# W298/Surtr

Measured on AMD Instinct MI355X. Metric: fragments/sec, higher is better.
Workload: dtype f32

## Files before the change

surtr_amd/csrc/surtr_hip.hip:

```cpp
#include <algorithm>
#include <cmath>
#include <cstdio>
#include <cstdlib>
#include <cstring>
#include <string>
#include <type_traits>
#include <vector>

#include "surtr_ctx.h"
#include "small_clip.h"
#ifndef SC_RESUME
#define SC_RESUME 1
#endif
#include "literal_clip.h"
#include "wave_clip.h"
#include "prep_sorted.h"

template <uint32_t LV, uint32_t LH>
struct alignas(16) LdsTopoT
{
    static_assert(LV % 16 == 0 && LH % 8 == 0, "clip_image copies 16-byte words into these arrays");
    static constexpr uint32_t kLV = LV, kLH = LH;
    alignas(16) uint16_t loff[LV];
    alignas(16) uint8_t llen[LV];
// ... 1812 lines not shown
    refit_fragments(HullFirst4{}, frags, counts, pool, A, forder, cap_frags, frag_status, piece_cpos, piece_cvo);
}

__global__ __launch_bounds__(SURTR_LANES) void k_refit_n(FragRec* __restrict__ frags, const surtr_counts* __restrict__ counts,
                                                      ScratchPool pool, Arena A, const uint32_t* __restrict__ forder, uint32_t cap_frags,
                                                      uint32_t* __restrict__ frag_status, const float* __restrict__ piece_cpos,
                                                      const uint32_t* __restrict__ piece_cvo, uint32_t limit, uint32_t* __restrict__ hull_ws)
{
    refit_fragments(HullLimited{limit, A.capV, hull_ws}, frags, counts, pool, A, forder, cap_frags, frag_status, piece_cpos, piece_cvo);
}

__global__ __launch_bounds__(SURTR_LANES) void k_hull_probe(const float* __restrict__ pts, uint32_t n, uint32_t limit, uint32_t* __restrict__ ws,
                                                         float* __restrict__ normals, uint32_t* __restrict__ out )
{
    __shared__ RhLds H;
    __shared__ ArgF slotF[SURTR_NWAVE];
    __shared__ ArgD slotD[SURTR_NWAVE];
    const int rc = rh_build(pts, n, n < limit ? n : limit, (float*)ws, ws + n, H, slotF, slotD);
    if (rc == 0)
        for (uint32_t i = threadIdx.x; i < 3u * H.nLive; i += group_size()) normals[i] = (&H.nrm[0][0])[i];
    if (threadIdx.x == 0) { out[0] = (uint32_t)rc; out[1] = rc == 0 ? H.nLive : 0u; }
}


__device__ __forceinline__ bool on_right(const float* a, const float* b, const float* c, float nx, float ny, float nz)
{
    const float ux = b[0] - a[0], uy = b[1] - a[1], uz = b[2] - a[2];
    const float wx = c[0] - a[0], wy = c[1] - a[1], wz = c[2] - a[2];
    const float cx = uy * wz - uz * wy, cy = uz * wx - ux * wz, cz = ux * wy - uy * wx;
    return dot3(cx, cy, cz, nx, ny, nz) > 0.f;
}

template <class LP>
__device__ __attribute__((always_inline)) static inline uint32_t ear_clip_face(const float* pos, const LP* loop, int N, int32_t* tmp, uint32_t* out)
{
    if (N <= 2) return 0;
    if (N == 3) { out[0] = loop[0]; out[1] = loop[1]; out[2] = loop[2]; return 3; }
    const float* A0 = pos + 3 * loop[0]; const float* B0 = pos + 3 * loop[1]; const float* C0 = pos + 3 * loop[2];
    float nx, ny, nz;
    {
        const float ux = B0[0] - A0[0], uy = B0[1] - A0[1], uz = B0[2] - A0[2];
        const float wx = C0[0] - A0[0], wy = C0[1] - A0[1], wz = C0[2] - A0[2];
        nx = uy * wz - uz * wy; ny = uz * wx - ux * wz; nz = ux * wy - uy * wx;
    }
    {
        float sx = 0.f, sy = 0.f, sz = 0.f;
        for (int v = 0; v < N; ++v)
        {
            const float* p = pos + 3 * loop[v]; const float* q = pos + 3 * loop[(v + 1) % N];
            const float ux = p[0] - A0[0], uy = p[1] - A0[1], uz = p[2] - A0[2];
            const float wx = q[0] - A0[0], wy = q[1] - A0[1], wz = q[2] - A0[2];
            sx = sx + (uy * wz - uz * wy); sy = sy + (uz * wx - ux * wz); sz = sz + (ux * wy - uy * wx);
        }
        if (dot3(sx, sy, sz, nx, ny, nz) < 0.f) { nx = -nx; ny = -ny; nz = -nz; }
    }
    int32_t* prv = tmp; int32_t* nxt = tmp + N; int32_t* rfx = tmp + 2 * N;
    for (int i = 0; i < N; ++i) { prv[i] = (i + N - 1) % N; nxt[i] = (i + 1) % N; }
    for (int i = 0; i < N; ++i)
        rfx[i] = on_right(pos + 3 * loop[prv[i]], pos + 3 * loop[i], pos + 3 * loop[nxt[i]], nx, ny, nz) ? 0 : 1;
    int skipped = 0, left = N, cur = 0;
    uint32_t at = 0;
    while (left > 3)
    {
        const int p = prv[cur], n = nxt[cur];
        bool ear = rfx[cur] == 0;
        if (ear)
        {
            const float* a = pos + 3 * loop[p]; const float* b = pos + 3 * loop[cur]; const float* c = pos + 3 * loop[n];
            for (int r = 0; r < N && ear; ++r)
            {
                if (!rfx[r]) continue;
                if (r == p || r == n) continue;
                const float* q = pos + 3 * loop[r];
                if ((q[0] == a[0] && q[1] == a[1] && q[2] == a[2]) || (q[0] == b[0] && q[1] == b[1] && q[2] == b[2])) continue;
                if (!on_right(a, b, q, nx, ny, nz)) continue;
                if (!on_right(b, c, q, nx, ny, nz)) continue;
                if (!on_right(c, a, q, nx, ny, nz)) continue;
                ear = false;
            }
        }
        if (ear)
        {
            out[at] = loop[p]; out[at + 1] = loop[cur]; out[at + 2] = loop[n];
            nxt[p] = n; prv[n] = p;
            const int adj[2] = {p, n};
            for (int k = 0; k < 2; ++k)
            {
                const int v = adj[k];
                if (!rfx[v]) continue;
                rfx[v] = on_right(pos + 3 * loop[prv[v]], pos + 3 * loop[v], pos + 3 * loop[nxt[v]], nx, ny, nz) ? 0 : 1;
            }
            at += 3; --left; skipped = 0;
        }
        else if (++skipped > left) return 0;
        cur = n;
    }
    out[at] = loop[prv[cur]]; out[at + 1] = loop[cur]; out[at + 2] = loop[nxt[cur]];
    return at + 3;
}

template <class LP>
__device__ __attribute__((always_inline)) static inline uint32_t ear_clip_small(const float* pos, const LP* loop, int N, uint32_t* out)
{
    if (N <= 2) return 0;
    if (N == 3) { out[0] = loop[0]; out[1] = loop[1]; out[2] = loop[2]; return 3; }
    auto P = [&](int i) -> const float* { return pos + 3 * (int)loop[i]; };
    const float* A0 = P(0); const float* B0 = P(1); const float* C0 = P(2);
    float nx, ny, nz;
    {
        const float ux = B0[0] - A0[0], uy = B0[1] - A0[1], uz = B0[2] - A0[2];
        const float wx = C0[0] - A0[0], wy = C0[1] - A0[1], wz = C0[2] - A0[2];
        nx = uy * wz - uz * wy; ny = uz * wx - ux * wz; nz = ux * wy - uy * wx;
    }
    {
        float sx = 0.f, sy = 0.f, sz = 0.f;
        for (int v = 0; v < N; ++v)
        {
            const float* p = P(v); const float* q = P((v + 1) % N);
            const float ux = p[0] - A0[0], uy = p[1] - A0[1], uz = p[2] - A0[2];
            const float wx = q[0] - A0[0], wy = q[1] - A0[1], wz = q[2] - A0[2];
            sx = sx + (uy * wz - uz * wy); sy = sy + (uz * wx - ux * wz); sz = sz + (ux * wy - uy * wx);
        }
        if (dot3(sx, sy, sz, nx, ny, nz) < 0.f) { nx = -nx; ny = -ny; nz = -nz; }
    }
    uint32_t prv = 0, nxt = 0, rfx = 0;
    auto get = [](uint32_t w, int i) -> int { return (int)((w >> (4 * i)) & 15u); };
    auto put = [](uint32_t& w, int i, int v) { w = (w & ~(15u << (4 * i))) | ((uint32_t)v << (4 * i)); };
    for (int i = 0; i < N; ++i) { put(prv, i, (i + N - 1) % N); put(nxt, i, (i + 1) % N); }
    for (int i = 0; i < N; ++i)
        if (!on_right(P(get(prv, i)), P(i), P(get(nxt, i)), nx, ny, nz)) rfx |= 1u << i;
    int skipped = 0, left = N, cur = 0;
    uint32_t at = 0;
    while (left > 3)
    {
        const int p = get(prv, cur), n = get(nxt, cur);
        bool ear = ((rfx >> cur) & 1u) == 0u;
        if (ear)
        {
            const float* a = P(p); const float* b = P(cur); const float* c = P(n);
            for (int r = 0; r < N && ear; ++r)
            {
                if (!((rfx >> r) & 1u)) continue;
                if (r == p || r == n) continue;
                const float* q = P(r);
                if ((q[0] == a[0] && q[1] == a[1] && q[2] == a[2]) || (q[0] == b[0] && q[1] == b[1] && q[2] == b[2])) continue;
                if (!on_right(a, b, q, nx, ny, nz)) continue;
                if (!on_right(b, c, q, nx, ny, nz)) continue;
                if (!on_right(c, a, q, nx, ny, nz)) continue;
                ear = false;
            }
        }
        if (ear)
        {
            out[at] = loop[p]; out[at + 1] = loop[cur]; out[at + 2] = loop[n];
            put(nxt, p, n); put(prv, n, p);
            const int adj[2] = {p, n};
            for (int k = 0; k < 2; ++k)
            {
                const int v = adj[k];
                if (!((rfx >> v) & 1u)) continue;
                if (on_right(P(get(prv, v)), P(v), P(get(nxt, v)), nx, ny, nz)) rfx &= ~(1u << v);
            }
            at += 3; --left; skipped = 0;
        }
        else if (++skipped > left) return 0;
        cur = n;
    }
    out[at] = loop[get(prv, cur)]; out[at + 1] = loop[cur]; out[at + 2] = loop[get(nxt, cur)];
    return at + 3;
}

#ifndef SURTR_EAR_WAVE_MAX
#define SURTR_EAR_WAVE_MAX 256u
#endif
#if SURTR_LANES == 64
template <class LP>
__device__ __attribute__((always_inline)) static inline uint32_t ear_clip_face_wave(const float* pos, const LP* loop, int N, uint32_t* out)
{
    const int lane = (int)lane_id();
    const bool mine = lane < N;
    const int32_t vid = (int32_t)loop[mine ? lane : 0];
    const float x = pos[3 * vid], y = pos[3 * vid + 1], z = pos[3 * vid + 2];
#ifdef SURTR_EAR_SHFL
#define EAR_BCAST(v, i) __shfl(v, i, 64)
#else
#define EAR_BCAST(v, i) lane_bcast(v, (uint32_t)(i))
#endif
    auto bx = [&](int i) { return EAR_BCAST(x, i); };
    auto by = [&](int i) { return EAR_BCAST(y, i); };
    auto bz = [&](int i) { return EAR_BCAST(z, i); };
    const float ax0 = bx(0), ay0 = by(0), az0 = bz(0);
    float nx, ny, nz;
    {
        const float ux = bx(1) - ax0, uy = by(1) - ay0, uz = bz(1) - az0;
        const float wx = bx(2) - ax0, wy = by(2) - ay0, wz = bz(2) - az0;
        nx = uy * wz - uz * wy; ny = uz * wx - ux * wz; nz = ux * wy - uy * wx;
    }
    {
        float sx = 0.f, sy = 0.f, sz = 0.f;
        for (int v = 0; v < N; ++v)
        {
            const int q = (v + 1) % N;
            const float ux = bx(v) - ax0, uy = by(v) - ay0, uz = bz(v) - az0;
            const float wx = bx(q) - ax0, wy = by(q) - ay0, wz = bz(q) - az0;
            sx = sx + (uy * wz - uz * wy); sy = sy + (uz * wx - ux * wz); sz = sz + (ux * wy - uy * wx);
        }
        if (dot3(sx, sy, sz, nx, ny, nz) < 0.f) { nx = -nx; ny = -ny; nz = -nz; }
    }
    int prv = (lane + N - 1) % N, nxt = (lane + 1) % N;
    auto right_of = [&](float ax, float ay, float az, float bx_, float by_, float bz_, float cx, float cy, float cz) {
        const float ux = bx_ - ax, uy = by_ - ay, uz = bz_ - az;
        const float wx = cx - ax, wy = cy - ay, wz = cz - az;
        const float kx = uy * wz - uz * wy, ky = uz * wx - ux * wz, kz = ux * wy - uy * wx;
        return dot3(kx, ky, kz, nx, ny, nz) > 0.f;
    };
    bool rfx = false;
    {
        const float px_ = __shfl(x, prv, 64), py_ = __shfl(y, prv, 64), pz_ = __shfl(z, prv, 64);
        const float qx = __shfl(x, nxt, 64), qy = __shfl(y, nxt, 64), qz = __shfl(z, nxt, 64);
        rfx = mine && !right_of(px_, py_, pz_, x, y, z, qx, qy, qz);
    }
    int skipped = 0, left = N, cur = 0;
    uint32_t at = 0;
    while (left > 3)
    {
        const int p = EAR_BCAST(prv, cur), n = EAR_BCAST(nxt, cur);
        const bool cur_reflex = EAR_BCAST((int)rfx, cur) != 0;
        bool ear = !cur_reflex;
        if (ear)
        {
            const float ax = bx(p), ay = by(p), az = bz(p);
            const float cx_ = bx(cur), cy_ = by(cur), cz_ = bz(cur);
            const float ex = bx(n), ey = by(n), ez = bz(n);
            bool inside = false;
            if (mine && rfx && lane != p && lane != n)
            {
                const bool same = (x == ax && y == ay && z == az) || (x == cx_ && y == cy_ && z == cz_);
                if (!same)
                    inside = right_of(ax, ay, az, cx_, cy_, cz_, x, y, z) && right_of(cx_, cy_, cz_, ex, ey, ez, x, y, z) &&
                             right_of(ex, ey, ez, ax, ay, az, x, y, z);
            }
            ear = __ballot(inside) == 0ull;
        }
        if (ear)
        {
            if (lane == 0) { out[at] = (uint32_t)loop[p]; out[at + 1] = (uint32_t)loop[cur]; out[at + 2] = (uint32_t)loop[n]; }
            if (lane == p) nxt = n;
            if (lane == n) prv = p;
            const int np = EAR_BCAST(prv, p), nn = EAR_BCAST(nxt, n);
            const float npx = bx(np), npy = by(np), npz = bz(np), nnx = bx(nn), nny = by(nn), nnz = bz(nn);
            const float ppx = bx(p), ppy = by(p), ppz = bz(p), qqx = bx(n), qqy = by(n), qqz = bz(n);
            if (lane == p && rfx) rfx = !right_of(npx, npy, npz, x, y, z, qqx, qqy, qqz);
            if (lane == n && rfx) rfx = !right_of(ppx, ppy, ppz, x, y, z, nnx, nny, nnz);
            at += 3; --left; skipped = 0;
        }
        else if (++skipped > left) return 0;
        cur = n;
    }
    {
        const int p = EAR_BCAST(prv, cur), n = EAR_BCAST(nxt, cur);
        if (lane == 0) { out[at] = (uint32_t)loop[p]; out[at + 1] = (uint32_t)loop[cur]; out[at + 2] = (uint32_t)loop[n]; }
    }
    return at + 3;
}

template <int K, class LP>
__device__ __attribute__((noinline)) static uint32_t ear_clip_face_wave_k(const float* pos, const LP* loop, int N, uint32_t* out)
{
    const int lane = (int)lane_id();
    float x[K], y[K], z[K]; int prv[K], nxt[K]; bool rfx[K], mine[K];
#pragma unroll
    for (int j = 0; j < K; ++j)
    {
        const int v = lane + 64 * j;
        mine[j] = v < N;
        const int32_t vid = (int32_t)loop[mine[j] ? v : 0];
        x[j] = pos[3 * vid]; y[j] = pos[3 * vid + 1]; z[j] = pos[3 * vid + 2];
        prv[j] = (v + N - 1) % N; nxt[j] = (v + 1) % N; rfx[j] = false;
    }
    auto bf = [&](const float (&a)[K], int i) -> float {
        const int jj = i >> 6; const uint32_t l = (uint32_t)(i & 63);
        float r = lane_bcast(a[0], l);
#pragma unroll
        for (int j = 1; j < K; ++j) { const float t = lane_bcast(a[j], l); r = jj == j ? t : r; }
        return r;
    };
    auto bi = [&](const int (&a)[K], int i) -> int {
        const int jj = i >> 6; const uint32_t l = (uint32_t)(i & 63);
        int r = lane_bcast(a[0], l);
#pragma unroll
        for (int j = 1; j < K; ++j) { const int t = lane_bcast(a[j], l); r = jj == j ? t : r; }
        return r;
    };
    auto bb = [&](const bool (&a)[K], int i) -> bool {
        const int jj = i >> 6; const uint32_t l = (uint32_t)(i & 63);
        int r = lane_bcast((int)a[0], l);
#pragma unroll
        for (int j = 1; j < K; ++j) { const int t = lane_bcast((int)a[j], l); r = jj == j ? t : r; }
        return r != 0;
    };
    const float ax0 = bf(x, 0), ay0 = bf(y, 0), az0 = bf(z, 0);
    float nx, ny, nz;
    {
        const float ux = bf(x, 1) - ax0, uy = bf(y, 1) - ay0, uz = bf(z, 1) - az0;
        const float wx = bf(x, 2) - ax0, wy = bf(y, 2) - ay0, wz = bf(z, 2) - az0;
        nx = uy * wz - uz * wy; ny = uz * wx - ux * wz; nz = ux * wy - uy * wx;
    }
    {
        float sx = 0.f, sy = 0.f, sz = 0.f;
        float px_ = ax0, py_ = ay0, pz_ = az0;
        for (int v = 0; v < N; ++v)
        {
            const int q = (v + 1) % N;
            const float qx = bf(x, q), qy = bf(y, q), qz = bf(z, q);
            const float ux = px_ - ax0, uy = py_ - ay0, uz = pz_ - az0;
            const float wx = qx - ax0, wy = qy - ay0, wz = qz - az0;
            sx = sx + (uy * wz - uz * wy); sy = sy + (uz * wx - ux * wz); sz = sz + (ux * wy - uy * wx);
            px_ = qx; py_ = qy; pz_ = qz;
        }
        if (dot3(sx, sy, sz, nx, ny, nz) < 0.f) { nx = -nx; ny = -ny; nz = -nz; }
    }
    auto right_of = [&](float ax, float ay, float az, float bx_, float by_, float bz_, float cx, float cy, float cz) {
        const float ux = bx_ - ax, uy = by_ - ay, uz = bz_ - az;
        const float wx = cx - ax, wy = cy - ay, wz = cz - az;
        const float kx = uy * wz - uz * wy, ky = uz * wx - ux * wz, kz = ux * wy - uy * wx;
        return dot3(kx, ky, kz, nx, ny, nz) > 0.f;
    };
#pragma unroll
    for (int j = 0; j < K; ++j)
    {
        float pxv = 0.f, pyv = 0.f, pzv = 0.f, qxv = 0.f, qyv = 0.f, qzv = 0.f;
#pragma unroll
        for (int s2 = 0; s2 < K; ++s2)
        {
            const float tx = __shfl(x[s2], prv[j] & 63, 64), ty = __shfl(y[s2], prv[j] & 63, 64), tz = __shfl(z[s2], prv[j] & 63, 64);
            if ((prv[j] >> 6) == s2) { pxv = tx; pyv = ty; pzv = tz; }
            const float ux = __shfl(x[s2], nxt[j] & 63, 64), uy = __shfl(y[s2], nxt[j] & 63, 64), uz = __shfl(z[s2], nxt[j] & 63, 64);
            if ((nxt[j] >> 6) == s2) { qxv = ux; qyv = uy; qzv = uz; }
        }
        rfx[j] = mine[j] && !right_of(pxv, pyv, pzv, x[j], y[j], z[j], qxv, qyv, qzv);
    }
    auto set_i = [&](int (&a)[K], int i, int val) {
#pragma unroll
        for (int j = 0; j < K; ++j) if (lane == (i & 63) && (i >> 6) == j) a[j] = val;
    };
    int skipped = 0, left = N, cur = 0;
    uint32_t at = 0;
    while (left > 3)
    {
        const int p = bi(prv, cur), n = bi(nxt, cur);
        bool ear = !bb(rfx, cur);
        if (ear)
        {
            const float ax = bf(x, p), ay = bf(y, p), az = bf(z, p);
            const float cx_ = bf(x, cur), cy_ = bf(y, cur), cz_ = bf(z, cur);
            const float ex = bf(x, n), ey = bf(y, n), ez = bf(z, n);
            bool inside = false;
#pragma unroll
            for (int j = 0; j < K; ++j)
            {
                const int v = lane + 64 * j;
                if (mine[j] && rfx[j] && v != p && v != n)
                {
                    const bool same = (x[j] == ax && y[j] == ay && z[j] == az) || (x[j] == cx_ && y[j] == cy_ && z[j] == cz_);
                    if (!same && right_of(ax, ay, az, cx_, cy_, cz_, x[j], y[j], z[j]) && right_of(cx_, cy_, cz_, ex, ey, ez, x[j], y[j], z[j]) &&
                        right_of(ex, ey, ez, ax, ay, az, x[j], y[j], z[j])) inside = true;
                }
            }
            ear = __ballot(inside) == 0ull;
        }
        if (ear)
        {
            if (lane == 0) { out[at] = (uint32_t)loop[p]; out[at + 1] = (uint32_t)loop[cur]; out[at + 2] = (uint32_t)loop[n]; }
            set_i(nxt, p, n);
            set_i(prv, n, p);
            const int np = bi(prv, p), nn = bi(nxt, n);
            const float npx = bf(x, np), npy = bf(y, np), npz = bf(z, np), nnx = bf(x, nn), nny = bf(y, nn), nnz = bf(z, nn);
            const float ppx = bf(x, p), ppy = bf(y, p), ppz = bf(z, p), qqx = bf(x, n), qqy = bf(y, n), qqz = bf(z, n);
#pragma unroll
            for (int j = 0; j < K; ++j)
            {
                const int v = lane + 64 * j;
                if (v == p && rfx[j]) rfx[j] = !right_of(npx, npy, npz, x[j], y[j], z[j], qqx, qqy, qqz);
                if (v == n && rfx[j]) rfx[j] = !right_of(ppx, ppy, ppz, x[j], y[j], z[j], nnx, nny, nnz);
            }
            at += 3; --left; skipped = 0;
        }
        else if (++skipped > left) return 0;
        cur = n;
    }
    {
        const int p = bi(prv, cur), n = bi(nxt, cur);
        if (lane == 0) { out[at] = (uint32_t)loop[p]; out[at + 1] = (uint32_t)loop[cur]; out[at + 2] = (uint32_t)loop[n]; }
    }
    return at + 3;
}
#endif

__global__ __launch_bounds__(SURTR_WG) __attribute__((amdgpu_waves_per_eu(4, 8))) void k_faces(FragRec* __restrict__ frags, const surtr_counts* __restrict__ counts,
                                                    FaceScratch FS, uint2* __restrict__ blkpool, uint32_t blk_per_wg,
                                                    Arena A, const uint32_t* __restrict__ forder, uint32_t cap_frags,
                                                    uint32_t fan, uint32_t* __restrict__ face_n, uint32_t* __restrict__ face_off,
                                                    int32_t* __restrict__ face_idx, uint32_t* __restrict__ frag_status,
                                                    const uint32_t* __restrict__ take_list, uint32_t* __restrict__ push_list)
{
    __shared__ Shared sh;
#ifndef SURTR_FL_V
#define SURTR_FL_V 1024
#define SURTR_FL_H 4096
#endif
    constexpr uint32_t FL_V = SURTR_FL_V, FL_H = SURTR_FL_H, FL_J = SURTR_FL_H / 2u;
    __shared__ uint16_t f_loff[FL_V]; __shared__ uint16_t f_llen[FL_V]; __shared__ uint16_t f_nbr[FL_H];
    struct IrrLds { uint8_t vis[FL_H]; uint32_t cov[FL_H]; };
    struct JumpLds { uint16_t k0[FL_J], k1[FL_J], x0[FL_J], x1[FL_J], d1[FL_J]; };
    struct EarLds { float pos[3 * FL_V]; uint16_t loop[FL_J]; };
    union FacesLds { IrrLds irr; JumpLds jmp; EarLds ear; };
    static_assert(sizeof(EarLds) <= sizeof(IrrLds), "the ear staging reuses the bytes of the face search");
    static_assert(sizeof(JumpLds) <= sizeof(IrrLds), "the pointer-jumping arrays fit the bytes of the irregular path");
    __shared__ FacesLds FU;
    uint8_t* const f_vis = FU.irr.vis; uint32_t* const f_cov = FU.irr.cov;
// ... 21 lines not shown
        const uint32_t f = sh.misc[7];
        if (f >= nf) break;
        FragRec fr = frags[f];
        const uint32_t n = fr.mv_n, H = fr.mh_n;
        STAMP_DECL;
#ifdef SURTR_STAMP
        const unsigned long long frag_t0 = __builtin_readcyclecounter();
        if (tid == 0) for (int q = 0; q < 16; ++q) sh.ph[q] = 0;
#endif
        if (H > HF)
        {
            if (tid == 0)
            {
                if (push_list != nullptr) push_list[atomicAdd(&A.cursors[CUR_FACES2_N], 1u)] = f;
                else atomicMax(&A.cursors[CUR_STATUS], (uint32_t)SURTR_E_CAPACITY);
            }
            continue;
        }
        const float* pos = A.pos + 3 * (size_t)fr.mv_off;
        const uint32_t* loff = A.loff + fr.mv_off; const uint32_t* llen = A.llen + fr.mv_off;
        const int32_t* nbr = A.nbr + fr.mh_off;
        const bool topo_lds = n <= FL_V && H <= FL_H && n < 0xFFFFu;
        const bool jump_lds = topo_lds && H <= FL_J;
        if (tid == 0) sh.flagBad = 0;
        if (topo_lds)
        {
            for (uint32_t v = tid; v < n; v += group_size()) { f_loff[v] = (uint16_t)(loff[v] - fr.mh_off); f_llen[v] = (uint16_t)llen[v]; }
            for (uint32_t e = tid; e < H; e += group_size()) f_nbr[e] = (uint16_t)nbr[e];
        }
        __syncthreads();
        auto gLO = [&](uint32_t v) -> uint32_t { return loff[v] - fr.mh_off; };
        auto gLN = [&](uint32_t v) -> uint32_t { return llen[v]; };
        auto lLO = [&](uint32_t v) -> uint32_t { return f_loff[v]; };
        auto lLN = [&](uint32_t v) -> uint32_t { return f_llen[v]; };
        auto successors = [&](auto LO, auto LN, const auto* NB, auto* NX, auto* KEY, int32_t* copy) {
            typedef typename std::remove_reference<decltype(NX[0])>::type XT;
            bool dup = false;
            for (uint32_t v = tid; v < n; v += group_size())
            {
                const uint32_t lo = LO(v), len = LN(v);
                for (uint32_t s = 0; s < len; ++s)
                {
                    const uint32_t b = (uint32_t)NB[lo + s];
                    for (uint32_t s2 = 0; s2 < s; ++s2) if ((uint32_t)NB[lo + s2] == b) dup = true;
                    const uint32_t lb = LO(b), nbq = LN(b);
                    uint32_t q = 0;
                    while (q < nbq && (uint32_t)NB[lb + q] != v) ++q;
// ... 157 lines not shown
                if (lensum > HF) return false;
                if (!irregular && lensum != H) pinched = true;
                const uint32_t nb = pinched ? 0u : (H + SURTR_LANES - 1u) >> SURTR_LSH;
                for (uint32_t b = wave_id(); b < nb; b += group_waves())
                {
                    const uint32_t e = (b << SURTR_LSH) + lane_id();
                    uint2 c = make_uint2(0u, 0u);
                    if (e < H) c = ownfn(e);
                    const uint2 ex = wave_excl2(c);
                    if (e < H && c.x)
                    {
                        const uint32_t fi = blk[b].x + ex.x, lo = blk[b].y + ex.y;
                        int32_t* loop = loopbuf + lo;
                        const uint32_t start = vertex_of(e);
                        uint32_t prev = start, curv = (uint32_t)NB[e];
                        uint32_t len = 1; loop[0] = (int32_t)start;
                        while (curv != start && len < c.y)
                        {
                            loop[len++] = (int32_t)curv;
                            const uint32_t nx = (uint32_t)face_next(NB + LO(curv), LN(curv), prev);
                            prev = curv; curv = nx;
                        }
                        faceLo[fi] = (int32_t)lo; faceLen[fi] = (int32_t)len;
                    }
                }
                return true;
            };
            auto owners_ranked = [&]() -> bool {
                auto vertex_of = [&](uint32_t e) -> uint32_t {
                    uint32_t lo_v = 0, hi_v = n;
                    while (hi_v - lo_v > 1) { const uint32_t mid = (lo_v + hi_v) >> 1; if (f_loff[mid] <= e) lo_v = mid; else hi_v = mid; }
                    return lo_v;
                };
                bool bad = false;
                for (uint32_t e = tid; e < H; e += group_size())
                {
                    const uint32_t t = (uint32_t)nxA[e], o = own16[e];
                    if (t >= H || own16[t] != o) { bad = true; continue; }
                    const uint32_t want = o == e ? 0u : (t == o ? 1u : (uint32_t)dist16[t] + 1u);
                    if ((uint32_t)dist16[e] != want) bad = true;
                }
                for (uint32_t v = tid; v < n; v += group_size())
                {
                    const uint32_t lo = f_loff[v], len = f_llen[v];
                    for (uint32_t s1 = 1; s1 < len; ++s1)
                        for (uint32_t s2 = 0; s2 < s1; ++s2) if (own16[lo + s1] == own16[lo + s2]) bad = true;
                }
                if (bad) sh.flagBad = 3;
                __syncthreads();
                if (sh.flagBad == 3) { pinched = true; return true; }
                auto ownfn = [&](uint32_t e) -> uint2 {
                    if ((uint32_t)own16[e] != e) return make_uint2(0u, 0u);
                    return make_uint2(1u, (uint32_t)dist16[(uint32_t)nxA[e]] + 1u);
                };
                scan_blocks(H, blk, sh, ownfn, nfaces, lensum);
                if (lensum != H) { pinched = true; return true; }
                uint16_t* lo_of = free16a; uint16_t* len_of = free16b;
                const uint32_t nb = (H + SURTR_LANES - 1u) >> SURTR_LSH;
                for (uint32_t b = wave_id(); b < nb; b += group_waves())
                {
                    const uint32_t e = (b << SURTR_LSH) + lane_id();
                    uint2 c = make_uint2(0u, 0u);
                    if (e < H) c = ownfn(e);
                    const uint2 ex = wave_excl2(c);
                    if (e < H && c.x)
                    {
                        const uint32_t fi = blk[b].x + ex.x, lo = blk[b].y + ex.y;
                        faceLo[fi] = (int32_t)lo; faceLen[fi] = (int32_t)c.y;
                        lo_of[e] = (uint16_t)lo; len_of[e] = (uint16_t)c.y;
                    }
                }
                __syncthreads();
                for (uint32_t e = tid; e < H; e += group_size())
                {
                    const uint32_t o = own16[e], d = dist16[e];
                    loopbuf[(uint32_t)lo_of[o] + (d == 0u ? 0u : (uint32_t)len_of[o] - d)] = (int32_t)vertex_of(e);
                }
                return true;
            };
            bool ok;
            if (own16 != nullptr && dist16 != nullptr) ok = owners_ranked();
            else if (own16 != nullptr) ok = owners(lLO, lLN, f_nbr, [&](uint32_t e) { return (uint32_t)own16[e] == e; });
            else if (topo_lds) ok = owners(lLO, lLN, f_nbr, [&](uint32_t e) { return kc[e] == (int32_t)e; });
            else ok = owners(gLO, gLN, nbr, [&](uint32_t e) { return kc[e] == (int32_t)e; });
            if (!ok) { failed = true; break; }
        }
        else
        {
            if (staged) { for (uint32_t e = tid; e < H; e += group_size()) f_vis[e] = 0; }
            else for (uint32_t e = tid; e < H; e += group_size()) keyA[e] = 0;
            __syncthreads();
// ... 6 lines not shown
                };
                uint32_t nfc = 0, lo = 0; bool bad = false;
                for (uint32_t i = 0; i < n && !bad; ++i)
                {
                    const uint32_t li = LO(i), ni = LN(i);
                    for (uint32_t s = 0; s < ni && !bad; ++s)
                    {
                        const uint32_t adj = NB[li + s];
                        if (visited[slot_of(i, adj)]) continue;
                        if (lo + 1 > HF || nfc >= HF) { bad = true; break; }
                        uint32_t len = 1; loopbuf[lo] = (int32_t)i;
                        uint32_t prev = i, curv = adj;
                        while (curv != i)
                        {
                            visited[slot_of(prev, curv)] = 1;
                            if (lo + len >= HF || len > H) { bad = true; break; }
                            loopbuf[lo + len++] = (int32_t)curv;
                            const uint32_t nx = face_next(NB + LO(curv), LN(curv), prev);
                            prev = curv; curv = nx;
                        }
                        if (bad) break;
                        visited[slot_of(prev, curv)] = 1;
                        faceLo[nfc] = (int32_t)lo; faceLen[nfc] = (int32_t)len; ++nfc; lo += len;
                    }
                }
                sh.misc[0] = nfc; sh.misc[1] = lo; sh.misc[2] = bad ? 1u : 0u;
            };
            if (tid == 0)
            {
                if (staged) extract([&](uint32_t v) { return (uint32_t)f_loff[v]; }, [&](uint32_t v) { return (uint32_t)f_llen[v]; }, f_nbr, f_vis);
                else extract([&](uint32_t v) { return loff[v] - fr.mh_off; }, [&](uint32_t v) { return llen[v]; }, nbr, keyA);
            }
            __syncthreads();
            nfaces = sh.misc[0]; lensum = sh.misc[1];
            const bool bad = sh.misc[2] != 0;
            __syncthreads();
            if (bad) { failed = true; break; }
        }
        __syncthreads();
        if (!pinched) break;
        irregular = true;
        if (tid == 0) sh.flagBad = 0;
        __syncthreads();
        }
        if (failed)
        {
            if (tid == 0)
            {
                frags[f].idx_off = 0; frags[f].idx_n = 0;
                if (frag_status == nullptr || atomicExch(&frag_status[f], (uint32_t)SURTR_E_TOPOLOGY) == 0u) atomicAdd(&A.cursors[CUR_FLAGGED_FRAGS], 1u);
            }
            continue;
        }
        if (face_n != nullptr)
        {
            for (uint32_t fi = tid; fi < nfaces; fi += group_size()) face_off[fi] = (uint32_t)faceLo[fi];
            for (uint32_t e = tid; e < lensum; e += group_size()) face_idx[e] = loopbuf[e];
            if (tid == 0) { face_off[nfaces] = lensum; face_n[0] = nfaces; face_n[1] = lensum; }
        }
        STAMP(62);
        const bool ear_lds = !fan && n <= FL_V && lensum <= FL_J;
        __syncthreads();
        if (ear_lds)
        {
            for (uint32_t i = tid; i < 3u * n; i += group_size()) FU.ear.pos[i] = pos[i];
            for (uint32_t e = tid; e < lensum; e += group_size()) FU.ear.loop[e] = (uint16_t)loopbuf[e];
            __syncthreads();
        }
        if (fan)
        {
            for (uint32_t fi = tid; fi < nfaces; fi += group_size())
            {
                const uint32_t lo = (uint32_t)faceLo[fi], len = (uint32_t)faceLen[fi];
                uint32_t* out = tri + 3u * (size_t)lo;
                const int32_t* loop = loopbuf + lo;
                uint32_t at = 0;
                for (uint32_t v = 1; v + 1u < len; ++v) { out[at] = (uint32_t)loop[0]; out[at + 1] = (uint32_t)loop[v]; out[at + 2] = (uint32_t)loop[v + 1]; at += 3u; }
                fcnt[fi] = at;
            }
        }
#if SURTR_LANES == 64
        for (uint32_t f0 = 0; f0 < (fan ? 0u : nfaces); f0 += SURTR_LANES)
        {
            const uint32_t fl = f0 + lane_id();
            uint32_t mylo = 0, mylen = 0;
            if (fl < nfaces) { mylo = (uint32_t)faceLo[fl]; mylen = (uint32_t)faceLen[fl]; }
            unsigned long long todo = __ballot(mylen >= 5u && mylen <= SURTR_EAR_WAVE_MAX);
            for (uint32_t ord = 0; todo != 0ull; todo &= todo - 1ull, ++ord)
            {
                if (ord % group_waves() != wave_id()) continue;
                const uint32_t src = (uint32_t)__builtin_ctzll(todo);
                const uint32_t lo = lane_bcast(mylo, src), len = lane_bcast(mylen, src);
                uint32_t cnt;
                if (len > 64u) cnt = ear_clip_face_wave_k<SURTR_EAR_WAVE_MAX / 64>(pos, (const int32_t*)loopbuf + lo, (int)len, tri + 3u * (size_t)lo);
                else if (ear_lds) cnt = ear_clip_face_wave((const float*)FU.ear.pos, (const uint16_t*)FU.ear.loop + lo, (int)len, tri + 3u * (size_t)lo);
                else cnt = ear_clip_face_wave(pos, (const int32_t*)loopbuf + lo, (int)len, tri + 3u * (size_t)lo);
                if (lane_id() == 0) fcnt[f0 + src] = cnt;
            }
        }
        __syncthreads();
        STAMP(63);
#endif
        for (uint32_t fi = tid; fi < (fan ? 0u : nfaces); fi += group_size())
        {
            const uint32_t lo = (uint32_t)faceLo[fi], len = (uint32_t)faceLen[fi];
#if SURTR_LANES == 64
            if (len >= 5u && len <= SURTR_EAR_WAVE_MAX) continue;
#endif
            uint32_t* out = tri + 3u * (size_t)lo;
            uint32_t cnt = 0u;
            if (len >= 3u && len <= 8u)
                cnt = ear_lds ? ear_clip_small((const float*)FU.ear.pos, (const uint16_t*)FU.ear.loop + lo, (int)len, out)
                              : ear_clip_small(pos, (const int32_t*)loopbuf + lo, (int)len, out);
            else if (len > 8u) cnt = ear_clip_face(pos, (const int32_t*)loopbuf + lo, (int)len, eartmp + 3 * (size_t)lo, out);
            fcnt[fi] = cnt;
#ifdef SURTR_STAMP
            if (len > 64u) { atomicAdd(&g_stamp[66], 1ull); atomicAdd(&g_stamp[67], (unsigned long long)len); }
#endif
        }
        __syncthreads();
        STAMP(64);
        auto cntfn = [&](uint32_t fi) -> uint2 { return make_uint2(fcnt[fi], 0u); };
        uint32_t nidx = 0, dum = 0;
        scan_blocks(nfaces, blk, sh, cntfn, nidx, dum);
        if (tid == 0) sh.misc[0] = atomicAdd(&A.cursors[CUR_I], nidx);
        __syncthreads();
        const uint32_t ioff = sh.misc[0];
        if ((uint64_t)ioff + nidx > A.capI) { if (tid == 0) atomicMax(&A.cursors[CUR_STATUS], (uint32_t)SURTR_E_CAPACITY); continue; }
        {
            const uint32_t nb = (nfaces + SURTR_LANES - 1u) >> SURTR_LSH;
            for (uint32_t b = wave_id(); b < nb; b += group_waves())
            {
                const uint32_t fi = (b << SURTR_LSH) + lane_id();
                uint2 c = make_uint2(0u, 0u);
                if (fi < nfaces) c = cntfn(fi);
                const uint2 ex = wave_excl2(c);
                if (fi < nfaces && c.x)
                {
                    const uint32_t* src = tri + 3u * (size_t)(uint32_t)faceLo[fi];
                    uint32_t* dst = A.idx + ioff + blk[b].x + ex.x;
                    for (uint32_t q = 0; q < c.x; ++q) dst[q] = src[q];
                }
            }
        }
        if (tid == 0) { frags[f].idx_off = ioff; frags[f].idx_n = nidx; }
        STAMP(65);
#ifdef SURTR_STAMP
        if (tid == 0)
        {
            const unsigned long long d = __builtin_readcyclecounter() - frag_t0;
            int bkt = 0; while ((d >> bkt) > 1 && bkt < 40) ++bkt; bkt = bkt < 12 ? 0 : bkt - 12; if (bkt > 15) bkt = 15;
            atomicAdd(&g_stamp2[32 + bkt], 1ull); atomicAdd(&g_stamp2[51], d);
            for (int q = 0; q < 6; ++q) atomicAdd(&g_stamp2[24 + q], sh.ph[(60 + q) & 15]);
            const unsigned long long old = atomicMax(&g_stamp2[48], d);
            if (d > old) { g_stamp2[49] = n; g_stamp2[50] = H; g_stamp2[55] = nfaces; for (int q = 0; q < 6; ++q) g_stamp2[56 + q] = sh.ph[(60 + q) & 15]; }
        }
#endif
    }
#ifdef SURTR_STAMP
    if (tid == 0) { const unsigned long long d = __builtin_readcyclecounter() - wg_t0f; atomicAdd(&g_stamp2[52], d); atomicMax(&g_stamp2[53], d); atomicAdd(&g_stamp2[54], 1ull); }
#endif
}

__global__ __launch_bounds__(SURTR_WG_WIDE) void k_out_scan(FragRec* __restrict__ frags, uint2* __restrict__ blk,
                                                       surtr_counts* __restrict__ counts, Arena A)
{
    __shared__ Shared sh;
    const uint32_t nf = counts->n_frag;
// ... 1190 lines not shown
{
    if (!counts) return 0;
    return blob_layout(*counts).total;
}

int surtr_event_pack_dev(surtr_ctx* ctx, void* dev_blob, size_t capacity)
{
    if (!ctx || !dev_blob) return SURTR_E_INVALID;
    if (!ctx->have_event) return SURTR_E_STATE;
    (void)hipSetDevice(ctx->device);
    if (ctx->last_current && blob_layout(ctx->last).total > capacity) return SURTR_E_CAPACITY;
    const uint32_t grid = std::max(1u, std::min(ctx->cap_frags, 2048u));
    hipStream_t st = ctx->stream;
    PROF_BEGIN(5);
    hipLaunchKernelGGL(k_pack, dim3(grid), dim3(SURTR_WG), 0, ctx->stream, ctx->d_frags, ctx->d_counts, ctx->arena, (char*)dev_blob,
                       capacity, (ctx->last_flags & SURTR_EVT_RENDER) ? 1u : 0u, ctx->d_frag_status,
                       ctx->color[0], ctx->color[1], ctx->color[2]);
    PROF_END(5);
    HIPCHK(hipGetLastError());
    return SURTR_OK;
}

#ifdef SURTR_STAMP
int surtr_debug_stamps2(unsigned long long out[64], int reset)
{
    if (hipMemcpyFromSymbol(out, HIP_SYMBOL(g_stamp2), sizeof(unsigned long long) * 64) != hipSuccess) return SURTR_E_HIP;
    if (reset) { unsigned long long z[64] = {}; (void)hipMemcpyToSymbol(HIP_SYMBOL(g_stamp2), z, sizeof(z)); }
    return SURTR_OK;
}
int surtr_debug_wplane(unsigned long long out[32], int reset)
{
#ifdef SURTR_STAMP
    if (hipMemcpyFromSymbol(out, HIP_SYMBOL(g_wplane), sizeof(unsigned long long) * 32) != hipSuccess) return SURTR_E_HIP;
    if (reset) { unsigned long long z[32] = {}; (void)hipMemcpyToSymbol(HIP_SYMBOL(g_wplane), z, sizeof(z)); }
    return SURTR_OK;
#else
    (void)out; (void)reset;
    return SURTR_E_STATE;
#endif
}

int surtr_debug_wneed(uint32_t* out, uint32_t n_words)
{
#ifdef SURTR_STAMP
    if (hipMemcpyFromSymbol(out, HIP_SYMBOL(g_wneed), sizeof(uint32_t) * std::min<uint32_t>(n_words, 4u * 8192u)) != hipSuccess) return SURTR_E_HIP;
    return SURTR_OK;
// ... 245 lines not shown
```

Baseline: 1.194 million.

## Write ear-clip triangles directly into final index buffer and fan-finish convex remainders

When every face has at least three vertices, the index-buffer range is reserved up front and each face's triangles are written straight to their final slot. This removes the scan-and-copy pass from the scratch triangle buffer. If any face stalls, it is marked with a sentinel and a fallback compaction pass runs. All ear-clip variants now stop clipping once no reflex vertices remain and fan-triangulate the rest, and modulo operations are replaced with comparisons. This adds stamp instrumentation, makes ear_clip_face noinline, and adds an in-place compaction path with a possible aliasing risk.

```diff
diff --git a/surtr_amd/csrc/surtr_hip.hip b/surtr_amd/csrc/surtr_hip.hip
--- a/surtr_amd/csrc/surtr_hip.hip
+++ b/surtr_amd/csrc/surtr_hip.hip
@@ -1858,6 +1858,20 @@
     if (threadIdx.x == 0) { out[0] = (uint32_t)rc; out[1] = rc == 0 ? H.nLive : 0u; }
 }
 
+#ifdef SURTR_STAMP
+__device__ unsigned long long g_stamp_faces[8];
+#define EAR_T0 const unsigned long long ear_t0 = __builtin_readcyclecounter()
+#define EAR_T1 const unsigned long long ear_t1 = __builtin_readcyclecounter()
+#define EAR_T2 do { if (lane == 0) { atomicAdd(&g_stamp_faces[2], ear_t1 - ear_t0); atomicAdd(&g_stamp_faces[3], __builtin_readcyclecounter() - ear_t1); atomicAdd(&g_stamp_faces[5], 1ull); } } while (0)
+#define FACES_T(name) const unsigned long long name = __builtin_readcyclecounter()
+#define FACES_ADD(i, d) do { if (lane_id() == 0) atomicAdd(&g_stamp_faces[i], (unsigned long long)(d)); } while (0)
+#else
+#define EAR_T0
+#define EAR_T1
+#define EAR_T2 do { } while (0)
+#define FACES_T(name)
+#define FACES_ADD(i, d) do { } while (0)
+#endif
 
 __device__ __forceinline__ bool on_right(const float* a, const float* b, const float* c, float nx, float ny, float nz)
 {
@@ -1867,8 +1881,10 @@
     return dot3(cx, cy, cz, nx, ny, nz) > 0.f;
 }
 
+#define EAR_STALLED 0xFFFFFFFFu
+
 template <class LP>
-__device__ __attribute__((always_inline)) static inline uint32_t ear_clip_face(const float* pos, const LP* loop, int N, int32_t* tmp, uint32_t* out)
+__device__ __attribute__((noinline)) static uint32_t ear_clip_face(const float* pos, const LP* loop, int N, int32_t* tmp, uint32_t* out)
 {
     if (N <= 2) return 0;
     if (N == 3) { out[0] = loop[0]; out[1] = loop[1]; out[2] = loop[2]; return 3; }
@@ -1883,7 +1899,7 @@
         float sx = 0.f, sy = 0.f, sz = 0.f;
         for (int v = 0; v < N; ++v)
         {
-            const float* p = pos + 3 * loop[v]; const float* q = pos + 3 * loop[(v + 1) % N];
+            const float* p = pos + 3 * loop[v]; const float* q = pos + 3 * loop[v + 1 == N ? 0 : v + 1];
             const float ux = p[0] - A0[0], uy = p[1] - A0[1], uz = p[2] - A0[2];
             const float wx = q[0] - A0[0], wy = q[1] - A0[1], wz = q[2] - A0[2];
             sx = sx + (uy * wz - uz * wy); sy = sy + (uz * wx - ux * wz); sz = sz + (ux * wy - uy * wx);
@@ -1891,12 +1907,16 @@
         if (dot3(sx, sy, sz, nx, ny, nz) < 0.f) { nx = -nx; ny = -ny; nz = -nz; }
     }
     int32_t* prv = tmp; int32_t* nxt = tmp + N; int32_t* rfx = tmp + 2 * N;
-    for (int i = 0; i < N; ++i) { prv[i] = (i + N - 1) % N; nxt[i] = (i + 1) % N; }
+    for (int i = 0; i < N; ++i) { prv[i] = i == 0 ? N - 1 : i - 1; nxt[i] = i + 1 == N ? 0 : i + 1; }
+    int nrfx = 0;
     for (int i = 0; i < N; ++i)
+    {
         rfx[i] = on_right(pos + 3 * loop[prv[i]], pos + 3 * loop[i], pos + 3 * loop[nxt[i]], nx, ny, nz) ? 0 : 1;
+        nrfx += rfx[i];
+    }
     int skipped = 0, left = N, cur = 0;
     uint32_t at = 0;
-    while (left > 3)
+    while (left > 3 && nrfx > 0)
     {
         const int p = prv[cur], n = nxt[cur];
         bool ear = rfx[cur] == 0;
@@ -1924,15 +1944,21 @@
             {
                 const int v = adj[k];
                 if (!rfx[v]) continue;
-                rfx[v] = on_right(pos + 3 * loop[prv[v]], pos + 3 * loop[v], pos + 3 * loop[nxt[v]], nx, ny, nz) ? 0 : 1;
+                if (on_right(pos + 3 * loop[prv[v]], pos + 3 * loop[v], pos + 3 * loop[nxt[v]], nx, ny, nz)) { rfx[v] = 0; --nrfx; }
             }
             at += 3; --left; skipped = 0;
         }
-        else if (++skipped > left) return 0;
+        else if (++skipped > left) { out[0] = EAR_STALLED; return 0; }
         cur = n;
     }
-    out[at] = loop[prv[cur]]; out[at + 1] = loop[cur]; out[at + 2] = loop[nxt[cur]];
-    return at + 3;
+    const uint32_t lp = (uint32_t)loop[prv[cur]];
+    for (int v = cur; left > 2; --left)
+    {
+        const int n = nxt[v];
+        out[at] = lp; out[at + 1] = loop[v]; out[at + 2] = loop[n];
+        at += 3; v = n;
+    }
+    return at;
 }
 
 template <class LP>
@@ -1952,7 +1978,7 @@
         float sx = 0.f, sy = 0.f, sz = 0.f;
         for (int v = 0; v < N; ++v)
         {
-            const float* p = P(v); const float* q = P((v + 1) % N);
+            const float* p = P(v); const float* q = P(v + 1 == N ? 0 : v + 1);
             const float ux = p[0] - A0[0], uy = p[1] - A0[1], uz = p[2] - A0[2];
             const float wx = q[0] - A0[0], wy = q[1] - A0[1], wz = q[2] - A0[2];
             sx = sx + (uy * wz - uz * wy); sy = sy + (uz * wx - ux * wz); sz = sz + (ux * wy - uy * wx);
@@ -1962,12 +1988,12 @@
     uint32_t prv = 0, nxt = 0, rfx = 0;
     auto get = [](uint32_t w, int i) -> int { return (int)((w >> (4 * i)) & 15u); };
     auto put = [](uint32_t& w, int i, int v) { w = (w & ~(15u << (4 * i))) | ((uint32_t)v << (4 * i)); };
-    for (int i = 0; i < N; ++i) { put(prv, i, (i + N - 1) % N); put(nxt, i, (i + 1) % N); }
+    for (int i = 0; i < N; ++i) { put(prv, i, i == 0 ? N - 1 : i - 1); put(nxt, i, i + 1 == N ? 0 : i + 1); }
     for (int i = 0; i < N; ++i)
         if (!on_right(P(get(prv, i)), P(i), P(get(nxt, i)), nx, ny, nz)) rfx |= 1u << i;
     int skipped = 0, left = N, cur = 0;
     uint32_t at = 0;
-    while (left > 3)
+    while (left > 3 && rfx != 0u)
     {
         const int p = get(prv, cur), n = get(nxt, cur);
         bool ear = ((rfx >> cur) & 1u) == 0u;
@@ -1999,11 +2025,17 @@
             }
             at += 3; --left; skipped = 0;
         }
-        else if (++skipped > left) return 0;
+        else if (++skipped > left) { out[0] = EAR_STALLED; return 0; }
         cur = n;
     }
-    out[at] = loop[get(prv, cur)]; out[at + 1] = loop[cur]; out[at + 2] = loop[get(nxt, cur)];
-    return at + 3;
+    const uint32_t lp = (uint32_t)loop[get(prv, cur)];
+    for (int v = cur; left > 2; --left)
+    {
+        const int n = get(nxt, v);
+        out[at] = lp; out[at + 1] = loop[v]; out[at + 2] = loop[n];
+        at += 3; v = n;
+    }
+    return at;
 }
 
 #ifndef SURTR_EAR_WAVE_MAX
@@ -2014,6 +2046,7 @@
 __device__ __attribute__((always_inline)) static inline uint32_t ear_clip_face_wave(const float* pos, const LP* loop, int N, uint32_t* out)
 {
     const int lane = (int)lane_id();
+    EAR_T0;
     const bool mine = lane < N;
     const int32_t vid = (int32_t)loop[mine ? lane : 0];
     const float x = pos[3 * vid], y = pos[3 * vid + 1], z = pos[3 * vid + 2];
@@ -2036,14 +2069,14 @@
         float sx = 0.f, sy = 0.f, sz = 0.f;
         for (int v = 0; v < N; ++v)
         {
-            const int q = (v + 1) % N;
+            const int q = v + 1 == N ? 0 : v + 1;
             const float ux = bx(v) - ax0, uy = by(v) - ay0, uz = bz(v) - az0;
             const float wx = bx(q) - ax0, wy = by(q) - ay0, wz = bz(q) - az0;
             sx = sx + (uy * wz - uz * wy); sy = sy + (uz * wx - ux * wz); sz = sz + (ux * wy - uy * wx);
         }
         if (dot3(sx, sy, sz, nx, ny, nz) < 0.f) { nx = -nx; ny = -ny; nz = -nz; }
     }
-    int prv = (lane + N - 1) % N, nxt = (lane + 1) % N;
+    int prv = lane == 0 ? N - 1 : lane - 1, nxt = lane + 1 >= N ? 0 : lane + 1;
     auto right_of = [&](float ax, float ay, float az, float bx_, float by_, float bz_, float cx, float cy, float cz) {
         const float ux = bx_ - ax, uy = by_ - ay, uz = bz_ - az;
         const float wx = cx - ax, wy = cy - ay, wz = cz - az;
@@ -2056,9 +2089,10 @@
         const float qx = __shfl(x, nxt, 64), qy = __shfl(y, nxt, 64), qz = __shfl(z, nxt, 64);
         rfx = mine && !right_of(px_, py_, pz_, x, y, z, qx, qy, qz);
     }
+    EAR_T1;
     int skipped = 0, left = N, cur = 0;
     uint32_t at = 0;
-    while (left > 3)
+    while (left > 3 && __ballot(rfx) != 0ull)
     {
         const int p = EAR_BCAST(prv, cur), n = EAR_BCAST(nxt, cur);
         const bool cur_reflex = EAR_BCAST((int)rfx, cur) != 0;
@@ -2083,6 +2117,7 @@
             if (lane == 0) { out[at] = (uint32_t)loop[p]; out[at + 1] = (uint32_t)loop[cur]; out[at + 2] = (uint32_t)loop[n]; }
             if (lane == p) nxt = n;
             if (lane == n) prv = p;
+            if (lane == cur) nxt = -1;
             const int np = EAR_BCAST(prv, p), nn = EAR_BCAST(nxt, n);
             const float npx = bx(np), npy = by(np), npz = bz(np), nnx = bx(nn), nny = by(nn), nnz = bz(nn);
             const float ppx = bx(p), ppy = by(p), ppz = bz(p), qqx = bx(n), qqy = by(n), qqz = bz(n);
@@ -2090,20 +2125,29 @@
             if (lane == n && rfx) rfx = !right_of(ppx, ppy, ppz, x, y, z, nnx, nny, nnz);
             at += 3; --left; skipped = 0;
         }
-        else if (++skipped > left) return 0;
+        else if (++skipped > left) { if (lane == 0) out[0] = EAR_STALLED; return 0; }
         cur = n;
     }
     {
-        const int p = EAR_BCAST(prv, cur), n = EAR_BCAST(nxt, cur);
-        if (lane == 0) { out[at] = (uint32_t)loop[p]; out[at + 1] = (uint32_t)loop[cur]; out[at + 2] = (uint32_t)loop[n]; }
-    }
-    return at + 3;
+        const int p = EAR_BCAST(prv, cur);
+        const unsigned long long alive = __ballot(mine && nxt >= 0);
+        const unsigned long long below = (1ull << lane) - 1ull, from = ~0ull << cur;
+        const uint32_t k = lane >= cur ? (uint32_t)__popcll(alive & from & below) : (uint32_t)__popcll(alive & from) + (uint32_t)__popcll(alive & below);
+        if (((alive >> lane) & 1ull) != 0ull && k + 2u < (uint32_t)left)
+        {
+            uint32_t* o = out + at + 3u * k;
+            o[0] = (uint32_t)loop[p]; o[1] = (uint32_t)loop[lane]; o[2] = (uint32_t)loop[nxt];
+        }
+    }
+    EAR_T2;
+    return at + 3u * (uint32_t)(left - 2);
 }
 
 template <int K, class LP>
 __device__ __attribute__((noinline)) static uint32_t ear_clip_face_wave_k(const float* pos, const LP* loop, int N, uint32_t* out)
 {
     const int lane = (int)lane_id();
+    EAR_T0;
     float x[K], y[K], z[K]; int prv[K], nxt[K]; bool rfx[K], mine[K];
 #pragma unroll
     for (int j = 0; j < K; ++j)
@@ -2112,7 +2156,7 @@
         mine[j] = v < N;
         const int32_t vid = (int32_t)loop[mine[j] ? v : 0];
         x[j] = pos[3 * vid]; y[j] = pos[3 * vid + 1]; z[j] = pos[3 * vid + 2];
-        prv[j] = (v + N - 1) % N; nxt[j] = (v + 1) % N; rfx[j] = false;
+        prv[j] = v == 0 ? N - 1 : v - 1; nxt[j] = v + 1 >= N ? 0 : v + 1; rfx[j] = false;
     }
     auto bf = [&](const float (&a)[K], int i) -> float {
         const int jj = i >> 6; const uint32_t l = (uint32_t)(i & 63);
@@ -2147,7 +2191,7 @@
         float px_ = ax0, py_ = ay0, pz_ = az0;
         for (int v = 0; v < N; ++v)
         {
-            const int q = (v + 1) % N;
+            const int q = v + 1 == N ? 0 : v + 1;
             const float qx = bf(x, q), qy = bf(y, q), qz = bf(z, q);
             const float ux = px_ - ax0, uy = py_ - ay0, uz = pz_ - az0;
             const float wx = qx - ax0, wy = qy - ay0, wz = qz - az0;
@@ -2180,9 +2224,16 @@
 #pragma unroll
         for (int j = 0; j < K; ++j) if (lane == (i & 63) && (i >> 6) == j) a[j] = val;
     };
+    EAR_T1;
     int skipped = 0, left = N, cur = 0;
     uint32_t at = 0;
-    while (left > 3)
+    auto any_reflex = [&]() -> bool {
+        bool r = false;
+#pragma unroll
+        for (int j = 0; j < K; ++j) r = r || rfx[j];
+        return __ballot(r) != 0ull;
+    };
+    while (left > 3 && any_reflex())
     {
         const int p = bi(prv, cur), n = bi(nxt, cur);
         bool ear = !bb(rfx, cur);
@@ -2210,6 +2261,7 @@
             if (lane == 0) { out[at] = (uint32_t)loop[p]; out[at + 1] = (uint32_t)loop[cur]; out[at + 2] = (uint32_t)loop[n]; }
             set_i(nxt, p, n);
             set_i(prv, n, p);
+            set_i(nxt, cur, -1);
             const int np = bi(prv, p), nn = bi(nxt, n);
             const float npx = bf(x, np), npy = bf(y, np), npz = bf(z, np), nnx = bf(x, nn), nny = bf(y, nn), nnz = bf(z, nn);
             const float ppx = bf(x, p), ppy = bf(y, p), ppz = bf(z, p), qqx = bf(x, n), qqy = bf(y, n), qqz = bf(z, n);
@@ -2222,16 +2274,85 @@
             }
             at += 3; --left; skipped = 0;
         }
-        else if (++skipped > left) return 0;
+        else if (++skipped > left) { if (lane == 0) out[0] = EAR_STALLED; return 0; }
         cur = n;
     }
     {
-        const int p = bi(prv, cur), n = bi(nxt, cur);
-        if (lane == 0) { out[at] = (uint32_t)loop[p]; out[at + 1] = (uint32_t)loop[cur]; out[at + 2] = (uint32_t)loop[n]; }
-    }
-    return at + 3;
-}
-#endif
+        const uint32_t lp = (uint32_t)loop[bi(prv, cur)];
+        const unsigned long long below = (1ull << lane) - 1ull;
+        unsigned long long alive[K];
+        uint32_t before_cur = 0, base = 0;
+#pragma unroll
+        for (int j = 0; j < K; ++j)
+        {
+            alive[j] = __ballot(mine[j] && nxt[j] >= 0);
+            if ((cur >> 6) == j) before_cur = base + (uint32_t)__popcll(alive[j] & ((1ull << (cur & 63)) - 1ull));
+            base += (uint32_t)__popcll(alive[j]);
+        }
+        base = 0;
+#pragma unroll
+        for (int j = 0; j < K; ++j)
+        {
+            const int v = lane + 64 * j;
+            const uint32_t before_v = base + (uint32_t)__popcll(alive[j] & below);
+            const uint32_t k = v >= cur ? before_v - before_cur : (uint32_t)left - before_cur + before_v;
+            if (((alive[j] >> lane) & 1ull) != 0ull && k + 2u < (uint32_t)left)
+            {
+                uint32_t* o = out + at + 3u * k;
+                o[0] = lp; o[1] = (uint32_t)loop[v]; o[2] = (uint32_t)loop[nxt[j]];
+            }
+            base += (uint32_t)__popcll(alive[j]);
+        }
+    }
+    EAR_T2;
+    return at + 3u * (uint32_t)(left - 2);
+}
+#endif
+
+struct FacesCompacted { uint32_t at, n; bool full; };
+__device__ __attribute__((noinline)) static FacesCompacted faces_compact(uint32_t nfaces, uint2* blk, Shared& sh, const int32_t* faceLo, const int32_t* faceLen,
+                                                                         const uint32_t* fcnt, uint32_t* tri, uint32_t* idx, uint32_t* cur_i, uint32_t capI, uint32_t placed_at)
+{
+    const bool placed = fcnt == nullptr;
+    auto src_of = [&](uint32_t fi) -> const uint32_t* {
+        const uint32_t lo = (uint32_t)faceLo[fi];
+        return placed ? idx + placed_at + 3u * (lo - 2u * fi) : tri + 3u * (size_t)lo;
+    };
+    auto cntfn = [&](uint32_t fi) -> uint2 {
+        if (!placed) return make_uint2(fcnt[fi], 0u);
+        return make_uint2(src_of(fi)[0] == EAR_STALLED ? 0u : 3u * ((uint32_t)faceLen[fi] - 2u), 0u);
+    };
+    uint32_t nidx = 0, dum = 0, at = placed_at;
+    scan_blocks(nfaces, blk, sh, cntfn, nidx, dum);
+    if (!placed)
+    {
+        if (threadIdx.x == 0) sh.misc[0] = atomicAdd(cur_i, nidx);
+        __syncthreads();
+        at = sh.misc[0];
+        if ((uint64_t)at + nidx > capI) return FacesCompacted{at, nidx, true};
+    }
+    uint32_t* const to = placed ? tri : idx + at;
+    const uint32_t nb = (nfaces + SURTR_LANES - 1u) >> SURTR_LSH;
+    for (uint32_t b = wave_id(); b < nb; b += group_waves())
+    {
+        const uint32_t fi = (b << SURTR_LSH) + lane_id();
+        uint2 c = make_uint2(0u, 0u);
+        if (fi < nfaces) c = cntfn(fi);
+        const uint2 ex = wave_excl2(c);
+        if (fi < nfaces && c.x)
+        {
+            const uint32_t* src = src_of(fi);
+            uint32_t* dst = to + blk[b].x + ex.x;
+            for (uint32_t q = 0; q < c.x; ++q) dst[q] = src[q];
+        }
+    }
+    if (placed)
+    {
+        __syncthreads();
+        for (uint32_t q = threadIdx.x; q < nidx; q += group_size()) idx[at + q] = tri[q];
+    }
+    return FacesCompacted{at, nidx, false};
+}
 
 __global__ __launch_bounds__(SURTR_WG) __attribute__((amdgpu_waves_per_eu(4, 8))) void k_faces(FragRec* __restrict__ frags, const surtr_counts* __restrict__ counts,
                                                     FaceScratch FS, uint2* __restrict__ blkpool, uint32_t blk_per_wg,
@@ -2299,7 +2420,7 @@
         const int32_t* nbr = A.nbr + fr.mh_off;
         const bool topo_lds = n <= FL_V && H <= FL_H && n < 0xFFFFu;
         const bool jump_lds = topo_lds && H <= FL_J;
-        if (tid == 0) sh.flagBad = 0;
+        if (tid == 0) { sh.flagBad = 0; sh.misc[3] = 0u; sh.misc[4] = 0u; }
         if (topo_lds)
         {
             for (uint32_t v = tid; v < n; v += group_size()) { f_loff[v] = (uint16_t)(loff[v] - fr.mh_off); f_llen[v] = (uint16_t)llen[v]; }
@@ -2503,6 +2624,7 @@
                             prev = curv; curv = nx;
                         }
                         faceLo[fi] = (int32_t)lo; faceLen[fi] = (int32_t)len;
+                        if (len < 3u) sh.misc[3] = 1u;
                     }
                 }
                 return true;
@@ -2548,6 +2670,7 @@
                     {
                         const uint32_t fi = blk[b].x + ex.x, lo = blk[b].y + ex.y;
                         faceLo[fi] = (int32_t)lo; faceLen[fi] = (int32_t)c.y;
+                        if (c.y < 3u) sh.misc[3] = 1u;
                         lo_of[e] = (uint16_t)lo; len_of[e] = (uint16_t)c.y;
                     }
                 }
@@ -2600,6 +2723,7 @@
                         if (bad) break;
                         visited[slot_of(prev, curv)] = 1;
                         faceLo[nfc] = (int32_t)lo; faceLen[nfc] = (int32_t)len; ++nfc; lo += len;
+                        if (len < 3u) sh.misc[3] = 1u;
                     }
                 }
                 sh.misc[0] = nfc; sh.misc[1] = lo; sh.misc[2] = bad ? 1u : 0u;
@@ -2618,7 +2742,7 @@
         __syncthreads();
         if (!pinched) break;
         irregular = true;
-        if (tid == 0) sh.flagBad = 0;
+        if (tid == 0) { sh.flagBad = 0; sh.misc[3] = 0u; }
         __syncthreads();
         }
         if (failed)
@@ -2637,14 +2761,25 @@
             if (tid == 0) { face_off[nfaces] = lensum; face_n[0] = nfaces; face_n[1] = lensum; }
         }
         STAMP(62);
+        FACES_T(ft_0);
         const bool ear_lds = !fan && n <= FL_V && lensum <= FL_J;
+        auto direct = [&]() -> bool { return !fan && SURTR_UNIFORM(sh.misc[3]) == 0u; };
+        if (direct() && tid == 0) sh.misc[5] = atomicAdd(&A.cursors[CUR_I], 3u * (lensum - 2u * nfaces));
         __syncthreads();
+        if (direct() && (uint64_t)sh.misc[5] + 3u * (lensum - 2u * nfaces) > A.capI) { if (tid == 0) atomicMax(&A.cursors[CUR_STATUS], (uint32_t)SURTR_E_CAPACITY); continue; }
+        auto out_of = [&](uint32_t fi, uint32_t lo) -> uint32_t* { return direct() ? A.idx + SURTR_UNIFORM(sh.misc[5]) + 3u * (lo - 2u * fi) : tri + 3u * (size_t)lo; };
+        auto count_of = [&](uint32_t fi, uint32_t cnt) {
+            if (!direct()) fcnt[fi] = cnt;
+            else if (cnt == 0u) sh.misc[4] = 1u;
+        };
         if (ear_lds)
         {
             for (uint32_t i = tid; i < 3u * n; i += group_size()) FU.ear.pos[i] = pos[i];
             for (uint32_t e = tid; e < lensum; e += group_size()) FU.ear.loop[e] = (uint16_t)loopbuf[e];
             __syncthreads();
         }
+        FACES_T(ft_1);
+        FACES_ADD(0, ft_1 - ft_0);
         if (fan)
         {
             for (uint32_t fi = tid; fi < nfaces; fi += group_size())
@@ -2660,23 +2795,29 @@
 #if SURTR_LANES == 64
         for (uint32_t f0 = 0; f0 < (fan ? 0u : nfaces); f0 += SURTR_LANES)
         {
+            FACES_T(ft_b0);
             const uint32_t fl = f0 + lane_id();
             uint32_t mylo = 0, mylen = 0;
             if (fl < nfaces) { mylo = (uint32_t)faceLo[fl]; mylen = (uint32_t)faceLen[fl]; }
             unsigned long long todo = __ballot(mylen >= 5u && mylen <= SURTR_EAR_WAVE_MAX);
+            FACES_ADD(1, __builtin_readcyclecounter() - ft_b0);
             for (uint32_t ord = 0; todo != 0ull; todo &= todo - 1ull, ++ord)
             {
                 if (ord % group_waves() != wave_id()) continue;
                 const uint32_t src = (uint32_t)__builtin_ctzll(todo);
                 const uint32_t lo = lane_bcast(mylo, src), len = lane_bcast(mylen, src);
+                uint32_t* const out = out_of(f0 + src, lo);
                 uint32_t cnt;
-                if (len > 64u) cnt = ear_clip_face_wave_k<SURTR_EAR_WAVE_MAX / 64>(pos, (const int32_t*)loopbuf + lo, (int)len, tri + 3u * (size_t)lo);
-                else if (ear_lds) cnt = ear_clip_face_wave((const float*)FU.ear.pos, (const uint16_t*)FU.ear.loop + lo, (int)len, tri + 3u * (size_t)lo);
-                else cnt = ear_clip_face_wave(pos, (const int32_t*)loopbuf + lo, (int)len, tri + 3u * (size_t)lo);
-                if (lane_id() == 0) fcnt[f0 + src] = cnt;
-            }
-        }
+                if (len > 64u) cnt = ear_clip_face_wave_k<SURTR_EAR_WAVE_MAX / 64>(pos, (const int32_t*)loopbuf + lo, (int)len, out);
+                else if (ear_lds) cnt = ear_clip_face_wave((const float*)FU.ear.pos, (const uint16_t*)FU.ear.loop + lo, (int)len, out);
+                else cnt = ear_clip_face_wave(pos, (const int32_t*)loopbuf + lo, (int)len, out);
+                if (lane_id() == 0) count_of(f0 + src, cnt);
+            }
+        }
+        FACES_T(ft_e0);
         __syncthreads();
+        FACES_ADD(4, __builtin_readcyclecounter() - ft_e0);
+        FACES_ADD(6, __builtin_readcyclecounter() - ft_0);
         STAMP(63);
 #endif
         for (uint32_t fi = tid; fi < (fan ? 0u : nfaces); fi += group_size())
@@ -2685,43 +2826,28 @@
 #if SURTR_LANES == 64
             if (len >= 5u && len <= SURTR_EAR_WAVE_MAX) continue;
 #endif
-            uint32_t* out = tri + 3u * (size_t)lo;
+            uint32_t* out = out_of(fi, lo);
             uint32_t cnt = 0u;
             if (len >= 3u && len <= 8u)
                 cnt = ear_lds ? ear_clip_small((const float*)FU.ear.pos, (const uint16_t*)FU.ear.loop + lo, (int)len, out)
                               : ear_clip_small(pos, (const int32_t*)loopbuf + lo, (int)len, out);
             else if (len > 8u) cnt = ear_clip_face(pos, (const int32_t*)loopbuf + lo, (int)len, eartmp + 3 * (size_t)lo, out);
-            fcnt[fi] = cnt;
+            count_of(fi, cnt);
 #ifdef SURTR_STAMP
             if (len > 64u) { atomicAdd(&g_stamp[66], 1ull); atomicAdd(&g_stamp[67], (unsigned long long)len); }
 #endif
         }
         __syncthreads();
         STAMP(64);
-        auto cntfn = [&](uint32_t fi) -> uint2 { return make_uint2(fcnt[fi], 0u); };
-        uint32_t nidx = 0, dum = 0;
-        scan_blocks(nfaces, blk, sh, cntfn, nidx, dum);
-        if (tid == 0) sh.misc[0] = atomicAdd(&A.cursors[CUR_I], nidx);
-        __syncthreads();
-        const uint32_t ioff = sh.misc[0];
-        if ((uint64_t)ioff + nidx > A.capI) { if (tid == 0) atomicMax(&A.cursors[CUR_STATUS], (uint32_t)SURTR_E_CAPACITY); continue; }
-        {
-            const uint32_t nb = (nfaces + SURTR_LANES - 1u) >> SURTR_LSH;
-            for (uint32_t b = wave_id(); b < nb; b += group_waves())
-            {
-                const uint32_t fi = (b << SURTR_LSH) + lane_id();
-                uint2 c = make_uint2(0u, 0u);
-                if (fi < nfaces) c = cntfn(fi);
-                const uint2 ex = wave_excl2(c);
-                if (fi < nfaces && c.x)
-                {
-                    const uint32_t* src = tri + 3u * (size_t)(uint32_t)faceLo[fi];
-                    uint32_t* dst = A.idx + ioff + blk[b].x + ex.x;
-                    for (uint32_t q = 0; q < c.x; ++q) dst[q] = src[q];
-                }
-            }
-        }
-        if (tid == 0) { frags[f].idx_off = ioff; frags[f].idx_n = nidx; }
+        const bool placed = direct();
+        uint32_t nidx = placed ? 3u * (lensum - 2u * nfaces) : 0u, idx_at = placed ? sh.misc[5] : 0u;
+        if (!placed || sh.misc[4] != 0u)
+        {
+            const FacesCompacted c = faces_compact(nfaces, blk, sh, faceLo, faceLen, placed ? nullptr : fcnt, tri, A.idx, &A.cursors[CUR_I], A.capI, idx_at);
+            if (c.full) { if (tid == 0) atomicMax(&A.cursors[CUR_STATUS], (uint32_t)SURTR_E_CAPACITY); continue; }
+            idx_at = c.at; nidx = c.n;
+        }
+        if (tid == 0) { frags[f].idx_off = idx_at; frags[f].idx_n = nidx; }
         STAMP(65);
 #ifdef SURTR_STAMP
         if (tid == 0)
@@ -3958,6 +4084,12 @@
 }
 
 #ifdef SURTR_STAMP
+int surtr_debug_stamps_faces(unsigned long long out[8], int reset)
+{
+    if (hipMemcpyFromSymbol(out, HIP_SYMBOL(g_stamp_faces), sizeof(unsigned long long) * 8) != hipSuccess) return SURTR_E_HIP;
+    if (reset) { unsigned long long z[8] = {}; (void)hipMemcpyToSymbol(HIP_SYMBOL(g_stamp_faces), z, sizeof(z)); }
+    return SURTR_OK;
+}
 int surtr_debug_stamps2(unsigned long long out[64], int reset)
 {
     if (hipMemcpyFromSymbol(out, HIP_SYMBOL(g_stamp2), sizeof(unsigned long long) * 64) != hipSuccess) return SURTR_E_HIP;
```

Result: faster. 1.208 million (median of 6 runs) (+1.1%).
